# jorr3/Alphazero-4-player-chess

Measured on AMD Instinct MI355X. Metric: MCTS simulations/sec (whole node), 256 games×400 sims, 10-block ResNet, higher is better.
Workload: dtype fp16

## Files before the change

### alphazero-4-player-chess_amd/csrc/fpc_nn.h

```cpp
#pragma once
#include <hip/hip_runtime.h>

#include <algorithm>
#include <cstdlib>
#include <cstring>
#include <string>
#include <vector>

#include "fpc_tree_kernels.h"
#include "fpc_tower.h"
#include "fpc_towerw.h"

namespace fpc {

typedef __attribute__((ext_vector_type(8))) __bf16 bf16x8_t;
typedef __attribute__((ext_vector_type(8))) _Float16 f16x8_t;
typedef __attribute__((ext_vector_type(16))) float f32x16_t;
typedef __attribute__((ext_vector_type(4))) uint32_t u32x4_t;
typedef __attribute__((ext_vector_type(2))) uint32_t u32x2_t;
typedef __attribute__((ext_vector_type(4))) float f32x4_t;

template <int DT>
struct E16;
template <>
// ... 273 lines not shown
          if (q0 + 64 * u < chunks) {
            const u32x4_t x = xrow[q0 + 64 * u];
            a0 = Dot16<DT>::dot2(w[u][0], x[0], a0); a1 = Dot16<DT>::dot2(w[u][1], x[1], a1);
            a2 = Dot16<DT>::dot2(w[u][2], x[2], a2); a3 = Dot16<DT>::dot2(w[u][3], x[3], a3);
          }
        }
      }
      float a = (a0 + a1) + (a2 + a3);
      for (int off = 32; off >= 1; off >>= 1) a += __shfl_xor(a, off);
      if (lane == 0) ll[(size_t)g * FPC_MAX_MOVES + j] = bias[nsrc] + a;
    }
    p = pend;
  }
}

template <int DT>
__global__ void __launch_bounds__(64) k_value_tail(const uint16_t *Y, const float *w, float bias, int P, int R, int PP,
                                                   int n, float *out) {
  const int g = blockIdx.x;
  if (g >= n) return;
  const int lane = threadIdx.x & 63;
  float acc = 0.f;
  for (int idx = lane; idx < R * R * 32; idx += 64) {
    const int q = idx >> 5, ch = idx & 31;
    const long m = (long)g * PP + (q / R + 1) * P + (q % R + 1);
    acc += E16<DT>::to_f32(Y[m * 32 + ch]) * w[idx];
  }
  for (int off = 32; off >= 1; off >>= 1) acc += __shfl_xor(acc, off);
  if (lane == 0) out[g] = tanhf(acc + bias);
}

template <int DT>
__global__ void __launch_bounds__(64) k_nchw_to_grid(const float *x, int n, int R, int P, uint16_t *out) {
  const int g = blockIdx.x;
  if (g >= n) return;
  const int lane = threadIdx.x & 63, RR = R * R;
  for (int q = lane; q < RR; q += 64) {
    uint16_t *row = out + ((long)g * P * P + (q / R + 1) * P + (q % R + 1)) * 32;
    for (int c = 0; c < 32; ++c) row[c] = c < 24 ? E16<DT>::from_f32(x[((long)g * 24 + c) * RR + q]) : (uint16_t)0;
  }
}

struct BlobHeader {
  char magic[4];
  int32_t version, R, F, nblocks, dtype, A_ch, Np, Kp;
  int32_t fc_layout;
  int32_t pad[6];
};
static_assert(sizeof(BlobHeader) == 64, "header is 64 bytes");

struct ConvW {
  uint16_t *w = nullptr;
  float *b = nullptr;
  int cin = 0, cout_pad = 0;
};

struct NN {
  bool loaded = false;
  DevCfg dc{};
  int Gmax = 0, dtype = 0, F = 0, nblocks = 0, P = 0, PP = 0, Np = 0, Kp = 0, Mrows = 0, guard = 64, Gpad = 0;
  hipStream_t stream = nullptr;
  std::vector<void *> allocs;
  uint16_t *in16 = nullptr;
  uint16_t *act[3] = {nullptr, nullptr, nullptr};
  uint16_t *yv = nullptr;
  uint16_t *xfc = nullptr;
  float *d_logits = nullptr;
  float *d_stats = nullptr;
  float *d_value = nullptr;
  ConvW stem, pconv, vconv;
  std::vector<ConvW> c1, c2;
  uint16_t *fcw = nullptr;
  float *fcb = nullptr, *vw = nullptr;
  float *fc_part = nullptr;
  int fc_G1 = 0, fc_s1 = FC_SPLITK, fc_s2 = FC_SPLITK;
  int fc_layout = 1;
  int fc_gw = 256;
  unsigned char *towerW = nullptr;
  unsigned char *stemW = nullptr;
  float *towerB = nullptr;
  bool use_tower = false;
  int tower_waves = 8;
  bool tower_compact = true;
  int towerw_rows = 1;
  bool use_towerw = false;
  void (*mark_fn)(void *, int) = nullptr;
  void *mark_ctx = nullptr;
  float vb = 0.f;
  bool attr_conv[2][3] = {{false, false, false}, {false, false, false}}, attr_tower[2] = {false, false}, attr_towerw[2] = {false, false}, attr_fc[2] = {false, false}, attr_gemv = false;

  template <class T>
  int dmalloc(T **p, size_t count, std::string *err) {
    void *q = nullptr;
    if (hipMalloc(&q, count * sizeof(T)) != hipSuccess) { *err = "hipMalloc failed in NN (" + std::to_string(count * sizeof(T)) + " bytes)"; return FPC_ENOMEM; }
    (void)hipMemset(q, 0, count * sizeof(T));
    allocs.push_back(q);
    *p = (T *)q;
    return 0;
  }

  int init(const DevCfg &c, int max_games, int nn_dtype, hipStream_t s, std::string *) {
    dc = c; Gmax = max_games; dtype = nn_dtype ? 1 : 0; stream = s;
    P = c.R + 2; PP = P * P;
    Mrows = ((max_games * PP + CONV_BM - 1) / CONV_BM) * CONV_BM;
    Gpad = ((max_games + 255) / 256) * 256;
    return 0;
  }
  void destroy() {
    for (void *p : allocs) (void)hipFree(p);
    allocs.clear();
    loaded = false;
    fcw2 = nullptr; d_ll = nullptr;
  }
  uint16_t *input16() { return in16 + (size_t)guard * 32; }
  const fpc_board *in_boards = nullptr;
  const int *in_leaf_slot = nullptr, *in_leaf_turn = nullptr;
  int in_board_stride = 0;
  bool takes_boards() const { return use_tower || use_towerw; }
  void set_board_input(const fpc_board *b, int stride, const int *slot, const int *turn) { in_boards = b; in_board_stride = stride; in_leaf_slot = slot; in_leaf_turn = turn; }
  uint16_t one16() const { return dtype ? 0x3C00 : 0x3F80; }
  float *logits() { return d_logits; }
  float *stats() { return d_stats; }
  float *value() { return d_value; }
  uint16_t *fcw2 = nullptr;
  float *d_ll = nullptr;
  float *legal_logits() { return d_ll; }

  static int plan_fcw(int Np, int Kp, int cus) {
    const int groups = Np / FCW_COLS, stages = Kp / 64;
    int best = 0;
    for (int sk = 1; sk <= 2 * FC_SPLITK && groups * sk <= cus; ++sk)
      if (stages % sk == 0 && stages / sk >= 4) best = sk;
    return best;
  }
  void plan_fc() {
    if (fc_layout == 2) { fc_G1 = Np / FCW_COLS; fc_s2 = fc_s1; return; }
    fc_s1 = FC_SPLITK;
    const int groups = Np / 256, ks = Kp / 16, mt = (Gmax + 255) / 256;
    fc_s2 = (ks % (2 * FC_SPLITK * 8) == 0 && ks / (2 * FC_SPLITK) / 4 >= 4) ? 2 * FC_SPLITK : FC_SPLITK;
    fc_G1 = groups;
    if (fc_s2 == FC_SPLITK) return;
    int cus = 256;
    hipDeviceProp_t prop;
    int dev = 0;
    (void)hipGetDevice(&dev);
    if (hipGetDeviceProperties(&prop, dev) == hipSuccess && prop.multiProcessorCount > 0) cus = prop.multiProcessorCount;
    long best = -1;
    std::vector<long> fin(cus);
    for (int g1 = groups; g1 >= 0; --g1) {
      std::fill(fin.begin(), fin.end(), 0L);
      for (int y = 0; y < mt; ++y)
        for (int id = 0, nb = g1 * FC_SPLITK + (groups - g1) * fc_s2; id < nb; ++id) {
          auto it = std::min_element(fin.begin(), fin.end());
          *it += id < g1 * FC_SPLITK ? 2 : 1;
        }
      const long span = *std::max_element(fin.begin(), fin.end());
      if (best < 0 || span < best) { best = span; fc_G1 = g1; }
    }
  }

  int load(const void *blob, uint64_t nbytes, std::string *err) {
    if (nbytes < sizeof(BlobHeader)) { *err = "weight blob too small"; return FPC_EWEIGHTS; }
    BlobHeader h;
    memcpy(&h, blob, sizeof(h));
    if (memcmp(h.magic, "FPCW", 4) || h.version != 3) { *err = "bad weight blob magic/version (this engine reads version 3; version 2 carried the retired 32x32x16 policy-Linear order: export again)"; return FPC_EWEIGHTS; }
    if (h.R != dc.R || h.A_ch != dc.A_ch) { *err = "weight blob is for a different board size"; return FPC_EWEIGHTS; }
    if (h.dtype != dtype) { *err = "weight blob dtype differs from engine nn_dtype"; return FPC_EWEIGHTS; }
    if (h.fc_layout < 1 || h.fc_layout > 2) { *err = "unknown policy-Linear weight layout in weight blob (1 = k_fc16, 2 = k_fcw)"; return FPC_EWEIGHTS; }
    if (h.F % 64 || h.F < 64 || h.F > 512 || h.nblocks < 0 || h.Np % (h.fc_layout == 2 ? FCW_COLS : 256) || h.Kp % 512 || h.Kp < 1024 || h.Np < dc.A || h.Kp < dc.A) {
      *err = "unsupported network shape in weight blob (hidden must be a multiple of 64, Np of 256 -- 384 for fc_layout 2 --, Kp of 512)";
      return FPC_EWEIGHTS;
    }
    int fcw_split = 0;
    if (h.fc_layout == 2) {
      int cus = 256, dev = 0;
      hipDeviceProp_t prop;
      (void)hipGetDevice(&dev);
      if (hipGetDeviceProperties(&prop, dev) == hipSuccess && prop.multiProcessorCount > 0) cus = prop.multiProcessorCount;
      fcw_split = plan_fcw(h.Np, h.Kp, cus);
      if (!fcw_split) { *err = "weight blob fc_layout 2 (k_fcw): no one-round K-split for this shape on this device; export with fc_layout 1"; return FPC_EWEIGHTS; }
    }
    destroy();
    F = h.F; nblocks = h.nblocks; Np = h.Np; Kp = h.Kp;
    fc_layout = h.fc_layout;
    fc_gw = fc_layout == 2 ? FCW_COLS : 256;
    if (fc_layout == 2) fc_s1 = fcw_split;
    const unsigned char *base = (const unsigned char *)blob;
    uint64_t off = sizeof(BlobHeader);
    int rc = 0;
    auto take = [&](void **dev, uint64_t bytes) -> int {
      off = (off + 63) & ~63ull;
      if (off + bytes > nbytes) { *err = "weight blob truncated"; return FPC_EWEIGHTS; }
      unsigned char *d = nullptr;
      if ((rc = dmalloc(&d, bytes, err))) return rc;
      if (hipMemcpy(d, base + off, bytes, hipMemcpyHostToDevice) != hipSuccess) { *err = "weight upload failed"; return FPC_ENODEVICE; }
      off += bytes;
      *dev = d;
      return 0;
    };
    auto conv = [&](ConvW &cw, int cin, int cout_pad) -> int {
      cw.cin = cin; cw.cout_pad = cout_pad;
      if ((rc = take((void **)&cw.w, (uint64_t)9 * cout_pad * cin * 2))) return rc;
      return take((void **)&cw.b, (uint64_t)cout_pad * 4);
    };
    const int Fp = (F + GEMM_BN - 1) / GEMM_BN * GEMM_BN;
    if ((rc = conv(stem, 32, Fp))) return rc;
    c1.assign(nblocks, ConvW()); c2.assign(nblocks, ConvW());
    for (int i = 0; i < nblocks; ++i) { if ((rc = conv(c1[i], F, Fp)) || (rc = conv(c2[i], F, Fp))) return rc; }
    if ((rc = conv(pconv, F, 128))) return rc;
    if ((rc = conv(vconv, F, 128))) return rc;
    if ((rc = take((void **)&fcw, (uint64_t)Np * Kp * 2)) || (rc = take((void **)&fcb, (uint64_t)Np * 4))) return rc;
    if ((rc = take((void **)&vw, (uint64_t)dc.RR * 32 * 4))) return rc;
    off = (off + 63) & ~63ull;
    if (off + 4 > nbytes) { *err = "weight blob truncated"; return FPC_EWEIGHTS; }
    memcpy(&vb, base + off, 4);
    const size_t rows = (size_t)Mrows + 2 * guard;
    if ((rc = dmalloc(&in16, rows * 32, err))) return rc;
    for (auto &a : act) if ((rc = dmalloc(&a, rows * F, err))) return rc;
    if ((rc = dmalloc(&yv, rows * 32, err))) return rc;
    if ((rc = dmalloc(&xfc, (size_t)Gpad * Kp, err))) return rc;
    if ((rc = dmalloc(&fc_part, (size_t)2 * FC_SPLITK * Gpad * Np, err))) return rc;
    plan_fc();
    if ((rc = dmalloc(&d_logits, (size_t)Gmax * dc.A, err))) return rc;
    if ((rc = dmalloc(&d_stats, (size_t)Gmax * SM_MAXCH * SM_REC, err))) return rc;
    if ((rc = dmalloc(&d_value, (size_t)Gmax, err))) return rc;
    use_tower = use_towerw = false;
    const bool dev = getenv("FPC_DEV_KNOBS") && atoi(getenv("FPC_DEV_KNOBS")) != 0;
    auto knob = [dev](const char *name, int dflt) { const char *v = dev ? getenv(name) : nullptr; return v ? atoi(v) : dflt; };
    const bool no_tower = knob("FPC_NO_TOWER", 0) != 0;
    tower_waves = knob("FPC_TOWER_WAVES", 8);
    tower_compact = knob("FPC_TOWER_COMPACT", 1) != 0;
    if (F == 256 && !no_tower) {
      use_towerw = true;
      towerw_rows = knob("FPC_TOWERW_ROWS", 1);
    } else if (F == 128 && !no_tower) {
      const int kw = knob("FPC_TOWERW", -1);
      use_towerw = kw < 0 ? dc.R != 14 : kw != 0;
      use_tower = !use_towerw;
    }
    const int layers = 2 * nblocks + 2;
    if (use_towerw) {
      const int slab = tww_slab(F), ksn = F / 32, tiles = F / 16;
      if ((rc = dmalloc(&towerW, ((size_t)layers * 9 * ksn + TWW_PAD_SLABS) * slab, err)) || (rc = dmalloc(&stemW, (size_t)9 * slab, err)) ||
          (rc = dmalloc(&towerB, (size_t)layers * 256, err))) return rc;
      auto prep = [&](const ConvW &cw, int layer) {
        hipLaunchKernelGGL(k_towerw_prep, dim3((9 * ksn * tiles * 64 + 255) / 256), dim3(256), 0, stream, (const uint16_t *)cw.w,
                           towerW + (size_t)layer * 9 * ksn * slab, 9, cw.cout_pad, F, tiles);
        (void)hipMemcpyAsync(towerB + (size_t)layer * 256, cw.b, (size_t)std::min(cw.cout_pad, F) * 4, hipMemcpyDeviceToDevice, stream);
      };
      for (int i = 0; i < nblocks; ++i) { prep(c1[i], 2 * i); prep(c2[i], 2 * i + 1); }
      prep(vconv, 2 * nblocks);
      prep(pconv, 2 * nblocks + 1);
      hipLaunchKernelGGL(k_towerw_prep, dim3((9 * tiles * 64 + 255) / 256), dim3(256), 0, stream, (const uint16_t *)stem.w, stemW, 9, stem.cout_pad, 32, tiles);
      if (hipStreamSynchronize(stream) != hipSuccess || hipGetLastError() != hipSuccess) { *err = "k_towerw_prep failed"; return FPC_ENODEVICE; }
    } else if (use_tower) {
      if ((rc = dmalloc(&towerW, (size_t)(layers * 9 + 3) * TW_TAP, err)) || (rc = dmalloc(&stemW, (size_t)9 * TW_STEM_TAP, err)) ||
          (rc = dmalloc(&towerB, (size_t)layers * 256, err))) return rc;
      auto prep = [&](const ConvW &cw, int layer) {
        hipLaunchKernelGGL(k_tower_prep, dim3((9 * 128 * 16 + 255) / 256), dim3(256), 0, stream, (const uint16_t *)cw.w,
                           towerW + (size_t)layer * 9 * TW_TAP, 9, 128);
        (void)hipMemcpyAsync(towerB + (size_t)layer * 256, cw.b, 128 * 4, hipMemcpyDeviceToDevice, stream);
      };
      for (int i = 0; i < nblocks; ++i) { prep(c1[i], 2 * i); prep(c2[i], 2 * i + 1); }
      prep(vconv, 2 * nblocks);
      prep(pconv, 2 * nblocks + 1);
      hipLaunchKernelGGL(k_tower_prep, dim3((9 * 128 * 4 + 255) / 256), dim3(256), 0, stream, (const uint16_t *)stem.w, stemW, 9, 32);
      if (hipStreamSynchronize(stream) != hipSuccess) { *err = "k_tower_prep failed"; return FPC_ENODEVICE; }
    }
    loaded = true;
    return 0;
  }

  template <int DT, int CINC>
  int launch_conv_c(const ConvArgs &g, int M, std::string *err) {
    constexpr int BKS = CINC < 64 ? CINC : 64;
    constexpr int IMG = (CONV_BM + 2 * CONV_HMAX) * CINC * 2;
    constexpr int lds = (IMG > CONV_BM * 64 * 4 ? IMG : CONV_BM * 64 * 4) + 3 * CONV_BN * BKS * 2 + CONV_BM;
    bool &attr = attr_conv[DT][CINC == 32 ? 0 : CINC == 64 ? 1 : 2];
    if (!attr) {
      (void)hipFuncSetAttribute(reinterpret_cast<const void *>(&k_conv3x3<DT, CINC>), hipFuncAttributeMaxDynamicSharedMemorySize, lds);
      attr = true;
    }
    dim3 grid(M / CONV_BM, g.cout_pad / CONV_BN), block(CONV_THREADS);
    hipLaunchKernelGGL((k_conv3x3<DT, CINC>), grid, block, lds, stream, g);
    const hipError_t le = hipGetLastError();
    if (le != hipSuccess) { *err = std::string("k_conv3x3 launch failed: ") + hipGetErrorString(le); return FPC_ENODEVICE; }
    return 0;
  }
  template <int DT>
  int launch_conv(const ConvArgs &g, int M, std::string *err) {
    if (g.P + 1 > CONV_HMAX) { *err = "board too large for the conv halo"; return FPC_EINVAL; }
    if (g.cin == 32) return launch_conv_c<DT, 32>(g, M, err);
    if (g.cin == 64) return launch_conv_c<DT, 64>(g, M, err);
    if (g.cin % 128 == 0) return launch_conv_c<DT, 128>(g, M, err);
    *err = "unsupported conv input width";
    return FPC_EINVAL;
  }

  template <int DT>
  int forward_t(int n, float *logits_out, float *value_out, std::string *err) {
    int rc;
    const int M = ((n * PP + CONV_BM - 1) / CONV_BM) * CONV_BM;
    auto conv = [&](const ConvW &cw, const uint16_t *in, int in_ld, const uint16_t *res, uint16_t *out, int out_ld, int n_valid, int mode) -> int {
      ConvArgs g{};
      g.X = in + (size_t)guard * in_ld; g.W = cw.w; g.bias = cw.b;
      g.Res = res ? res + (size_t)guard * out_ld : nullptr;
      g.out = mode == 1 ? out : out + (size_t)guard * out_ld;
      g.ldx = in_ld; g.ldo = out_ld; g.cin = cw.cin; g.cout_pad = cw.cout_pad;
      g.P = P; g.R = dc.R; g.PP = PP; g.n_valid = n_valid; g.m_valid = n; g.mode = mode;
      return launch_conv<DT>(g, M, err);
    };
    int cur = 0;
    if (use_tower || use_towerw) {
      TowerArgs t{};
      t.boards = in_boards; t.leaf_slot = in_leaf_slot; t.leaf_turn = in_leaf_turn; t.board_stride = in_board_stride; t.one16 = one16();
      in_boards = nullptr;
      t.in16 = in16 + (size_t)guard * 32; t.Wstem = stemW; t.bstem = stem.b; t.Wt = towerW; t.bt = towerB;
      t.xfc = xfc; t.vw = vw; t.value = value_out; t.vb = vb;
      t.L = 2 * nblocks; t.P = P; t.R = dc.R; t.PP = PP; t.NR = PP - P; t.T0 = (P + 1) / 16; t.n_games = n; t.Kp = Kp; t.A_ch = dc.A_ch; t.rules = dc.rules;
#if defined(TW_STAMPS) || defined(TWW_STAMPS)
      static unsigned long long *d_stamps = nullptr;
      if (!d_stamps) { (void)hipMalloc(&d_stamps, 2 * 8 * 16 * 8); }
      (void)hipMemsetAsync(d_stamps, 0, 2 * 8 * 16 * 8, stream);
      t.stamps = d_stamps;
#endif
      const int mt = dc.R <= 8 ? 3 : dc.R <= 11 ? 5 : 7;
      bool &attr = attr_tower[DT];
      if (!attr) {
        (void)hipFuncSetAttribute(reinterpret_cast<const void *>(&k_tower<DT, 3, false, 4>), hipFuncAttributeMaxDynamicSharedMemorySize, TW_LDS);
        (void)hipFuncSetAttribute(reinterpret_cast<const void *>(&k_tower<DT, 5, false, 4>), hipFuncAttributeMaxDynamicSharedMemorySize, TW_LDS);
        (void)hipFuncSetAttribute(reinterpret_cast<const void *>(&k_tower<DT, 7, false, 4>), hipFuncAttributeMaxDynamicSharedMemorySize, TW_LDS);
        (void)hipFuncSetAttribute(reinterpret_cast<const void *>(&k_tower<DT, 7, true, 4>), hipFuncAttributeMaxDynamicSharedMemorySize, TW_LDS);
        (void)hipFuncSetAttribute(reinterpret_cast<const void *>(&k_tower<DT, 7, true, 8>), hipFuncAttributeMaxDynamicSharedMemorySize, TW_LDS);
        (void)hipFuncSetAttribute(reinterpret_cast<const void *>(&k_tower<DT, 3, false, 8>), hipFuncAttributeMaxDynamicSharedMemorySize, TW_LDS);
        (void)hipFuncSetAttribute(reinterpret_cast<const void *>(&k_tower<DT, 5, false, 8>), hipFuncAttributeMaxDynamicSharedMemorySize, TW_LDS);
        (void)hipFuncSetAttribute(reinterpret_cast<const void *>(&k_tower<DT, 7, false, 8>), hipFuncAttributeMaxDynamicSharedMemorySize, TW_LDS);
        (void)hipFuncSetAttribute(reinterpret_cast<const void *>(&k_towerc<DT>), hipFuncAttributeMaxDynamicSharedMemorySize, TW_LDS);
        attr = true;
      }
      if (use_towerw) {
        bool &aw = attr_towerw[DT];
        if (!aw) {
#define FPC_TWW_ATTR(F_, MT_) (void)hipFuncSetAttribute(reinterpret_cast<const void *>(&k_towerw<DT, F_, MT_>), hipFuncAttributeMaxDynamicSharedMemorySize, tww_lds(F_))
#define FPC_TWW_ATTRS(F_) FPC_TWW_ATTR(F_, 2); FPC_TWW_ATTR(F_, 3); FPC_TWW_ATTR(F_, 4); FPC_TWW_ATTR(F_, 5); FPC_TWW_ATTR(F_, 6); FPC_TWW_ATTR(F_, 7)
          FPC_TWW_ATTRS(256); FPC_TWW_ATTRS(128);
#define FPC_TWW_ATTR1(F_, MT_) (void)hipFuncSetAttribute(reinterpret_cast<const void *>(&k_towerw<DT, F_, MT_, true>), hipFuncAttributeMaxDynamicSharedMemorySize, tww_lds(F_))
          FPC_TWW_ATTR1(128, 4); FPC_TWW_ATTR1(256, 4); FPC_TWW_ATTR1(256, 6); FPC_TWW_ATTR1(256, 7); FPC_TWW_ATTR1(256, 8);
          FPC_TWW_ATTR1(256, 9); FPC_TWW_ATTR1(256, 11); FPC_TWW_ATTR1(256, 13);
#undef FPC_TWW_ATTR1
          aw = true;
        }
        const int mtw = tww_mt(dc.R);
        if (mtw < 2 || mtw > 7) { *err = "k_towerw: board size outside 8..14"; return FPC_EINVAL; }
#define FPC_TWW_GO(F_, MT_) hipLaunchKernelGGL((k_towerw<DT, F_, MT_>), dim3(n), dim3(TWW_THREADS), tww_lds(F_), stream, t)
#define FPC_TWW_GOS(F_) switch (mtw) { case 2: FPC_TWW_GO(F_, 2); break; case 3: FPC_TWW_GO(F_, 3); break; case 4: FPC_TWW_GO(F_, 4); break; \
                                       case 5: FPC_TWW_GO(F_, 5); break; case 6: FPC_TWW_GO(F_, 6); break; default: FPC_TWW_GO(F_, 7); break; }
        const int tiles = tww_tiles(dc.R);
        const bool onerow = tiles <= 4 || (F == 256 && towerw_rows != 2);
#define FPC_TWW_GO1(F_, MT_) hipLaunchKernelGGL((k_towerw<DT, F_, MT_, true>), dim3(n), dim3(TWW_THREADS), tww_lds(F_), stream, t)
        if (onerow && F == 128) FPC_TWW_GO1(128, 4);
        else if (onerow) {
          switch (tiles) {
            case 4: FPC_TWW_GO1(256, 4); break;   case 6: FPC_TWW_GO1(256, 6); break;   case 7: FPC_TWW_GO1(256, 7); break;
            case 8: FPC_TWW_GO1(256, 8); break;   case 9: FPC_TWW_GO1(256, 9); break;   case 11: FPC_TWW_GO1(256, 11); break;
            default: FPC_TWW_GO1(256, 13); break;
          }
        } else if (F == 256) { FPC_TWW_GOS(256) } else { FPC_TWW_GOS(128) }
#undef FPC_TWW_GO1
#undef FPC_TWW_GOS
#undef FPC_TWW_GO
      } else if (mt == 3 && tower_waves == 8) hipLaunchKernelGGL((k_tower<DT, 3, false, 8>), dim3(n), dim3(512), TW_LDS, stream, t);
      else if (mt == 3) hipLaunchKernelGGL((k_tower<DT, 3, false, 4>), dim3(n), dim3(256), TW_LDS, stream, t);
      else if (mt == 5 && tower_waves == 8) hipLaunchKernelGGL((k_tower<DT, 5, false, 8>), dim3(n), dim3(512), TW_LDS, stream, t);
      else if (mt == 5) hipLaunchKernelGGL((k_tower<DT, 5, false, 4>), dim3(n), dim3(256), TW_LDS, stream, t);
      else if (P != 16 && tower_waves == 8) hipLaunchKernelGGL((k_tower<DT, 7, false, 8>), dim3(n), dim3(512), TW_LDS, stream, t);
      else if (P != 16) hipLaunchKernelGGL((k_tower<DT, 7, false, 4>), dim3(n), dim3(256), TW_LDS, stream, t);
      else if (tower_waves == 8 && tower_compact && dc.R == 14) hipLaunchKernelGGL((k_towerc<DT>), dim3(n), dim3(512), TW_LDS, stream, t);
      else if (tower_waves == 8) hipLaunchKernelGGL((k_tower<DT, 7, true, 8>), dim3(n), dim3(512), TW_LDS, stream, t);
      else hipLaunchKernelGGL((k_tower<DT, 7, true, 4>), dim3(n), dim3(256), TW_LDS, stream, t);
      const hipError_t le = hipGetLastError();
      if (le != hipSuccess) { *err = std::string("k_tower launch failed: ") + hipGetErrorString(le); return FPC_ENODEVICE; }
#if defined(TW_STAMPS) || defined(TWW_STAMPS)
      if (getenv("FPC_TW_STAMPS_FILE")) {
        unsigned long long h[2 * 8 * 16];
        (void)hipStreamSynchronize(stream);
        (void)hipMemcpy(h, t.stamps, sizeof(h), hipMemcpyDeviceToHost);
        if (FILE *f = fopen(getenv("FPC_TW_STAMPS_FILE"), "w")) {
          for (int i = 0; i < 2 * 8 * 16; ++i) fprintf(f, "%llu%c", h[i], i % 16 == 15 ? '\n' : ' ');
          fclose(f);
        }
      }
#endif
    } else if ((rc = conv(stem, in16, 32, nullptr, act[0], F, F, 0))) return rc;
    const bool fused = use_tower || use_towerw;
    for (int i = 0; i < nblocks && !fused; ++i) {
      const int t1 = (cur + 1) % 3, t2 = (cur + 2) % 3;
      if ((rc = conv(c1[i], act[cur], F, nullptr, act[t1], F, F, 0))) return rc;
      if ((rc = conv(c2[i], act[t1], F, act[cur], act[t2], F, F, 0))) return rc;
      cur = t2;
    }
    if (!fused) {
      if ((rc = conv(pconv, act[cur], F, nullptr, xfc, Kp, dc.A_ch, 1))) return rc;
      if ((rc = conv(vconv, act[cur], F, nullptr, yv, 32, 24, 0))) return rc;
    }
    if (mark_fn) mark_fn(mark_ctx, 2);
#if defined(TW_STRIP) && (TW_STRIP & 128)
    if (false) {
#else
    if (logits_out) {
#endif
      FcArgs f{};
      f.X = xfc; f.Wf = fcw; f.part = fc_part; f.Kp = Kp; f.Np = Np; f.ksteps = Kp / 16; f.Mtot = Gpad;
      f.G1 = fc_G1; f.s1 = fc_s1; f.s2 = fc_s2;
      const int mtiles = (n + 255) / 256;
      const int blocks = fc_G1 * fc_s1 + (Np / fc_gw - fc_G1) * fc_s2;
      bool &fattr = attr_fc[DT];
      if (!fattr) {
        (void)hipFuncSetAttribute(reinterpret_cast<const void *>(&k_fc16<DT>), hipFuncAttributeMaxDynamicSharedMemorySize, FC_LDS);
        (void)hipFuncSetAttribute(reinterpret_cast<const void *>(&k_fcw<DT>), hipFuncAttributeMaxDynamicSharedMemorySize, FCW_LDS);
        fattr = true;
      }
      if (fc_layout == 2) hipLaunchKernelGGL((k_fcw<DT>), dim3(blocks, mtiles), dim3(FC_THREADS), FCW_LDS, stream, f);
      else hipLaunchKernelGGL((k_fc16<DT>), dim3(blocks, mtiles), dim3(FC_THREADS), FC_LDS, stream, f);
      hipLaunchKernelGGL(k_fc_reduce, dim3((dc.A / 4 + 255) / 256, n), dim3(256), 0, stream, (const float *)fc_part, (const float *)fcb,
                         fc_G1, fc_s1, fc_s2, fc_gw, Gpad, dc.A, n, skip_dense ? (float *)nullptr : logits_out, d_stats);
      const hipError_t le = hipGetLastError();
      if (le != hipSuccess) { *err = std::string("k_fc launch failed: ") + hipGetErrorString(le); return FPC_ENODEVICE; }
    }
    if (!fused) hipLaunchKernelGGL((k_value_tail<DT>), dim3(n), dim3(64), 0, stream, (const uint16_t *)(yv + (size_t)guard * 32),
                       (const float *)vw, vb, P, dc.R, PP, n, value_out);
    if (hipGetLastError() != hipSuccess) { *err = "k_value_tail launch failed"; return FPC_ENODEVICE; }
    return 0;
  }

  bool skip_dense = false;
  int forward(int n, bool dense_logits, std::string *err) {
    skip_dense = !dense_logits;
    const int rc = dtype ? forward_t<1>(n, d_logits, d_value, err) : forward_t<0>(n, d_logits, d_value, err);
    skip_dense = false;
    return rc;
  }
  static_assert(2 * FC_SPLITK <= LOGIT_MAX_SLABS, "logit_at() requests at most LOGIT_MAX_SLABS slabs per column");
  LogitSrc logit_src(bool dense) const {
    if (dense) return LogitSrc{d_logits, nullptr, nullptr, 0, 0, 0, 0, 256};
    return LogitSrc{nullptr, fc_part, fcb, fc_G1, fc_s1, fc_s2, Gpad, fc_gw};
  }
  int ensure_legal_head(std::string *err) {
    if (fcw2) return 0;
    if (Gmax > GEMV_MAXG) { *err = "legal-only policy head supports at most " + std::to_string(GEMV_MAXG) + " games per engine"; return FPC_EINVAL; }
    int rc;
    if ((rc = dmalloc(&fcw2, (size_t)Np * Kp, err)) || (rc = dmalloc(&d_ll, (size_t)Gmax * FPC_MAX_MOVES, err))) return rc;
    const long chunks = (long)Np * (Kp / 8);
    if (dtype) hipLaunchKernelGGL((k_fc_unfrag<1>), dim3((unsigned)((chunks + 255) / 256)), dim3(256), 0, stream, (const uint16_t *)fcw, fcw2, Np, Kp);
    else hipLaunchKernelGGL((k_fc_unfrag<0>), dim3((unsigned)((chunks + 255) / 256)), dim3(256), 0, stream, (const uint16_t *)fcw, fcw2, Np, Kp);
    if (hipGetLastError() != hipSuccess) { *err = "k_fc_unfrag launch failed"; return FPC_ENODEVICE; }
    return 0;
  }
  int forward_legal(int n, const Tree &t, std::string *err) {
    int rc = ensure_legal_head(err);
    if (rc) return rc;
// ... 27 lines not shown
```

### alphazero-4-player-chess_amd/csrc/fpc_tower.h

```cpp
#pragma once
#include <hip/hip_runtime.h>

#include <type_traits>

#include "fpc_tree_kernels.h"

namespace fpc {

typedef __attribute__((ext_vector_type(8))) __bf16 t_bf16x8;
typedef __attribute__((ext_vector_type(8))) _Float16 t_f16x8;
typedef __attribute__((ext_vector_type(4))) float t_f32x4;
typedef __attribute__((ext_vector_type(2))) float t_f32x2;
typedef __attribute__((ext_vector_type(4))) uint32_t t_u32x4;
typedef __attribute__((ext_vector_type(2))) uint32_t t_u32x2;
typedef __attribute__((ext_vector_type(2))) short t_i16x2;

template <int DT>
struct M16;
template <>
struct M16<0> {
  static __device__ __forceinline__ t_f32x4 mfma(t_u32x4 a, t_u32x4 b, t_f32x4 c) {
    return __builtin_amdgcn_mfma_f32_16x16x32_bf16(__builtin_bit_cast(t_bf16x8, a), __builtin_bit_cast(t_bf16x8, b), c, 0, 0, 0);
  }
  static __device__ __forceinline__ uint32_t pack2(float lo, float hi) {
// ... 43 lines not shown
  const int *leaf_slot, *leaf_turn;
  int board_stride;
  uint16_t one16;
  const uint16_t *in16;
  const unsigned char *Wstem;
  const float *bstem;
  const unsigned char *Wt;
  const float *bt;
  uint16_t *xfc;
  const float *vw;
  float *value;
  float vb;
  int L, P, R, PP, NR, T0, n_games, Kp, A_ch;
  int rules;
  unsigned long long *stamps;
};

__device__ __forceinline__ void tw_dma_8k(const unsigned char *gsrc_uniform, uint32_t lane_off, uint32_t lds_addr_uniform) {
  uint32_t keep;
  asm volatile(
      "s_mov_b32 %0, m0\n\ts_mov_b32 m0, %3\n\ts_nop 0\n\t"
      "global_load_lds_dwordx4 %1, %2\n\ts_add_u32 m0, m0, 0x400\n\tv_add_u32 %1, 0x400, %1\n\t"
      "global_load_lds_dwordx4 %1, %2\n\ts_add_u32 m0, m0, 0x400\n\tv_add_u32 %1, 0x400, %1\n\t"
      "global_load_lds_dwordx4 %1, %2\n\ts_add_u32 m0, m0, 0x400\n\tv_add_u32 %1, 0x400, %1\n\t"
      "global_load_lds_dwordx4 %1, %2\n\ts_add_u32 m0, m0, 0x400\n\tv_add_u32 %1, 0x400, %1\n\t"
      "global_load_lds_dwordx4 %1, %2\n\ts_add_u32 m0, m0, 0x400\n\tv_add_u32 %1, 0x400, %1\n\t"
      "global_load_lds_dwordx4 %1, %2\n\ts_add_u32 m0, m0, 0x400\n\tv_add_u32 %1, 0x400, %1\n\t"
      "global_load_lds_dwordx4 %1, %2\n\ts_add_u32 m0, m0, 0x400\n\tv_add_u32 %1, 0x400, %1\n\t"
      "global_load_lds_dwordx4 %1, %2\n\t"
      "s_mov_b32 m0, %0"
      : "=&s"(keep), "+v"(lane_off) : "s"(gsrc_uniform), "s"(lds_addr_uniform) : "memory", "scc");
}
__device__ __forceinline__ void tw_dma_4k(const unsigned char *gsrc_uniform, uint32_t lane_off, uint32_t lds_addr_uniform) {
  uint32_t keep;
  asm volatile(
      "s_mov_b32 %0, m0\n\ts_mov_b32 m0, %3\n\ts_nop 0\n\t"
      "global_load_lds_dwordx4 %1, %2\n\ts_add_u32 m0, m0, 0x400\n\tv_add_u32 %1, 0x400, %1\n\t"
      "global_load_lds_dwordx4 %1, %2\n\ts_add_u32 m0, m0, 0x400\n\tv_add_u32 %1, 0x400, %1\n\t"
      "global_load_lds_dwordx4 %1, %2\n\ts_add_u32 m0, m0, 0x400\n\tv_add_u32 %1, 0x400, %1\n\t"
      "global_load_lds_dwordx4 %1, %2\n\t"
      "s_mov_b32 m0, %0"
      : "=&s"(keep), "+v"(lane_off) : "s"(gsrc_uniform), "s"(lds_addr_uniform) : "memory", "scc");
}
template <int OFF>
__device__ __forceinline__ void tw_dma_piece(const unsigned char *gsrc_uniform, uint32_t lane_off) {
  asm volatile("global_load_lds_dwordx4 %0, %1 offset:%2" : : "v"(lane_off), "s"(gsrc_uniform), "i"(OFF) : "memory");
}
__device__ __forceinline__ void tw_set_m0(uint32_t lds_addr_uniform) {
  asm volatile("s_mov_b32 m0, %0\n\ts_nop 0" : : "s"(lds_addr_uniform) : "memory");
}
__device__ __forceinline__ void tw_dma_256(const unsigned char *gsrc_uniform, uint32_t lane_off, uint32_t lds_addr_uniform) {
  uint32_t keep;
  asm volatile("s_mov_b32 %0, m0\n\ts_mov_b32 m0, %3\n\ts_nop 0\n\tglobal_load_lds_dword %1, %2\n\ts_mov_b32 m0, %0"
               : "=&s"(keep) : "v"(lane_off), "s"(gsrc_uniform), "s"(lds_addr_uniform) : "memory");
}

#ifdef TW_STAMPS
#define TW_STAMP(GT, I)                                                                                       \
  do {                                                                                                        \
    if (g.stamps && blockIdx.x == 0 && ((GT) == TW_STAMPS || (GT) == TW_STAMPS + 1)) {                        \
      const unsigned long long t_ = __builtin_amdgcn_s_memtime();                                             \
      if (lane == 0) g.stamps[(((GT) - TW_STAMPS) * 8 + wave) * 16 + (I)] = t_;                               \
    }                                                                                                         \
  } while (0)
#else
#define TW_STAMP(GT, I) do {} while (0)
#endif
#ifndef TW_AHEAD
#define TW_AHEAD 2
#endif
#ifndef TW_LOADERS
#define TW_LOADERS 1
#endif
#ifndef TW_STAGGER
#define TW_STAGGER 3
#endif
#ifndef TW_STRIP
#define TW_STRIP 0
#endif
#ifndef TWC_LOADER_TILES
#define TWC_LOADER_TILES 6
#endif

template <int DT, int MT, bool FAST, int NW, int LOAD, bool CMP = false>
__device__ __forceinline__ void tw_body(const TowerArgs &g) {
  static_assert(!CMP || (!FAST && NW == 8 && TW_LOADERS == 1 && MT == (LOAD == 2 ? TWC_LOADER_TILES : 13 - TWC_LOADER_TILES)), "compact form: 8 waves, 13 row tiles");
  constexpr int CR = 14, CZ = 16;
  constexpr int TB0 = LOAD == 2 ? 0 : TWC_LOADER_TILES;
  constexpr int NT = NW * 64;
  constexpr int WN = NW / 2;
  constexpr int CT = 8 / WN;
  constexpr int PIECES = 4 * LOAD;
  constexpr int DMA_PER_WAVE = PIECES * 1024;
  constexpr int MID = PIECES == 8 ? 4096 : 0;
  constexpr bool STREAM = TW_AHEAD == 2 && !(TW_STAGGER != 0 && NW == 8 && TW_LOADERS == 1);
  constexpr int STAG = (NW == 8 && TW_LOADERS == 1 && LOAD == 0) ? TW_STAGGER : 0;
  extern __shared__ __attribute__((aligned(16))) unsigned char smem[];
  unsigned char *const img = smem + TW_IMG0;
  unsigned char *const ring = smem + TW_RING;
  const float *const biasbuf = reinterpret_cast<const float *>(smem + TW_BIAS);
  float *const vred = reinterpret_cast<float *>(smem + TW_VRED);
  fpc_board *const lboard = reinterpret_cast<fpc_board *>(smem + TW_BOARD);
  const int tid = threadIdx.x, lane = tid & 63;
  const int wave = __builtin_amdgcn_readfirstlane(tid >> 6);
  const int wm = wave / WN, wn = wave % WN;
  const int li = lane & 15, lq = lane >> 4;
  const int game = blockIdx.x;
  const int P = g.P, NR = g.NR;

  int slot = 0, rot_k = 0;
  if (g.boards) {
    slot = g.leaf_slot[game];
    if (slot < 0) return;
    rot_k = first_leaf_turn(g.leaf_slot, g.leaf_turn, g.n_games);
  }

  const int rbase = CMP ? CZ + TB0 * 16 + li : (g.T0 + wm * MT) * 16 + li;
  uint32_t inmask = 0;
#pragma unroll
  for (int mt = 0; mt < MT; ++mt) {
    const int r = rbase + 16 * mt;
    if (CMP) {
      if (r - CZ < CR * CR) inmask |= 1u << mt;
    } else {
      const int pi = r / P, pj = r - pi * P;
      if (r < g.PP && pi >= 1 && pi <= g.R && pj >= 1 && pj <= g.R) inmask |= 1u << mt;
    }
  }
  auto colmask = [](int mt, int dx) -> uint64_t {
    uint32_t m16 = 0;
    for (int i = 0; i < 16; ++i)
      if (dx != 0 && ((TB0 + mt) * 16 + i) % CR == (dx < 0 ? 0 : CR - 1)) m16 |= 1u << i;
    const uint32_t m32 = m16 * 0x10001u;
    return ((uint64_t)m32 << 32) | m32;
  };
  auto lane_select = [](uint32_t a, uint32_t b, uint64_t m) -> uint32_t {
    uint32_t r;
    asm("v_cndmask_b32_e64 %0, %1, %2, %3" : "=v"(r) : "v"(a), "v"(b), "s"(m));
    return r;
  };
  const int bq = (lq >> 1) * 256 + (lq & 1) * 128;
  const int apart = (li >> 3) * 2048 + (li & 7) * 16 + bq;
  const int apart_s = (li >> 3) * 512 + (li & 7) * 16 + bq;
  const int cb64 = wn * (CT * 16);
  const int cb16 = (wn & 1) * 16;
  const bool vactive = wn < 2;

  for (int c = tid; c < (TW_IMG0 + TW_IMG) / 16; c += NT) reinterpret_cast<t_u32x4 *>(smem)[c] = t_u32x4{0u, 0u, 0u, 0u};
  unsigned char *const enc = smem + TW_ENC;
  const int enc_bytes = CMP ? 240 * 64 : ((NR + 7) >> 3) * 512;
  for (int c = tid; c < enc_bytes / 16; c += NT) reinterpret_cast<t_u32x4 *>(enc)[c] = t_u32x4{0u, 0u, 0u, 0u};
  {
    const t_u32x4 *src = reinterpret_cast<const t_u32x4 *>(g.Wstem);
    t_u32x4 *dst = reinterpret_cast<t_u32x4 *>(ring);
    for (int c = tid; c < 9 * TW_STEM_TAP / 16; c += NT) dst[c] = src[c];
  }
  t_f32x4 bst[CT];
#pragma unroll
  for (int ct = 0; ct < CT; ++ct) bst[ct] = *reinterpret_cast<const t_f32x4 *>(g.bstem + cb64 + ct * 16 + 4 * lq);
  __syncthreads();
  if (g.boards) {
    constexpr int WPB = (int)(sizeof(fpc_board) / 4);
    if (tid < WPB) reinterpret_cast<uint32_t *>(lboard)[tid] =
        reinterpret_cast<const uint32_t *>(g.boards + (size_t)game * g.board_stride + slot)[tid];
    __syncthreads();
    if (g.rules & FPC_RULES_ROTATION) rot_k = lboard->turn;
    for (int r = tid; r < (CMP ? CR * CR : g.PP); r += NT) {
      const int pi = CMP ? r / CR + 1 : r / P, pj = CMP ? r % CR + 1 : r - pi * P;
      if (pi < 1 || pi > g.R || pj < 1 || pj > g.R) continue;
      const uint8_t p = lboard->sq[rot90_src(g.R, rot_k, pi - 1, pj - 1)];
      if (!present(p)) continue;
      const int plane = piece_plane(p, lboard->turn, g.rules);
      *reinterpret_cast<uint16_t *>(enc + tw_lay(4, CMP ? CZ + r : r, plane >> 3) + (plane & 7) * 2) = g.one16;
    }
  } else if (CMP) {
    const uint16_t *src = g.in16 + (size_t)game * g.PP * 32;
    for (int c = tid; c < CR * CR * 4; c += NT) {
      const int q = c >> 2, j = c & 3;
      *reinterpret_cast<t_u32x4 *>(enc + tw_lay(4, CZ + q, j)) =
// ... 59 lines not shown
  auto open_tap = [&](int T) {
    issue_bias(T);
    if (LOAD == 0) return;
    dsrc = g.Wt + (size_t)T * TW_TAP + lw * DMA_PER_WAVE + MID;
    tw_set_m0((uint32_t)__builtin_amdgcn_readfirstlane(TW_RING + (T % 3) * TW_TAP + lw * DMA_PER_WAVE + MID));
  };
  auto piece = [&](auto i_c) {
    constexpr int I = decltype(i_c)::value;
    if (LOAD != 0) tw_dma_piece<I * 1024 - MID>(dsrc, dma_lane);
  };
  issue_tap(0);
  issue_tap(1);
  if (STREAM) {
    open_tap(2);
    piece(std::integral_constant<int, 0>{});
    if (LOAD == 2) piece(std::integral_constant<int, 1>{});
  }

  unsigned char *const dummy = smem + TW_DUMMY + lane * 8;
  unsigned char *const wbase = img + (rbase >> 3) * 2048 + (rbase & 7) * 16 + wn * (CT * 256) + (lane >> 5) * 128 + ((lane >> 4) & 1) * 8;
  auto epilogue = [&](auto res_c) {
    constexpr int RES = decltype(res_c)::value;
    if (TW_STRIP & 16) return;
#pragma unroll
    for (int mt = 0; mt < MT; ++mt) {
      unsigned char *dst = ((inmask >> mt) & 1u) ? wbase + mt * 4096 : dummy;
#pragma unroll
      for (int ct = 0; ct < CT; ++ct) {
        t_f32x4 v = acc[mt][ct];
        if (RES == 2) {
          v[0] += M16<DT>::lo(res[mt][ct][0]); v[1] += M16<DT>::hi(res[mt][ct][0]);
          v[2] += M16<DT>::lo(res[mt][ct][1]); v[3] += M16<DT>::hi(res[mt][ct][1]);
        }
        const t_u32x2 pk = t_u32x2{tw_relu2(M16<DT>::pack2(v[0], v[1])), tw_relu2(M16<DT>::pack2(v[2], v[3]))};
        if (RES != 0) res[mt][ct] = pk;
        *reinterpret_cast<t_u32x2 *>(((inmask >> mt) & 1u) ? dst + ct * 256 : dst) = pk;
      }
      __builtin_amdgcn_sched_barrier(0);
    }
  };
  const std::integral_constant<int, 0> c0{};
  const std::integral_constant<int, 1> c1{};
  const std::integral_constant<int, 2> c2{};
  const std::integral_constant<int, 3> c3{};
  epilogue(c1);
  if (TW_STRIP & 32) { asm volatile("s_waitcnt vmcnt(0)" ::: "memory"); return; }
  if (STREAM) asm volatile("s_waitcnt vmcnt(%0)" ::"n"(PIECES + LOAD) : "memory");
  else asm volatile("s_waitcnt vmcnt(0)" ::: "memory");
  __syncthreads();

  t_u32x4 fa[2][CT], fb[2][MT];
  int gt = 0;
  const unsigned char *wslot;
  const unsigned char *bbase;
  const unsigned char *blast;
  int boff[FAST ? 1 : MT];
  auto set_tap = [&](int tap, int cb) {
    wslot = ring + (gt % 3) * TW_TAP + cb * 256 + apart;
    const int shift = (tap / 3 - 1) * P + (tap % 3 - 1);
    if (FAST) {
      const int r = rbase + shift;
      bbase = img + (r >> 3) * 2048 + (r & 7) * 16 + bq;
      int rl = r + 16 * (MT - 1);
      rl = rl >= NR ? rl - NR : rl;
      blast = img + (rl >> 3) * 2048 + (rl & 7) * 16 + bq;
    } else if (CMP) {
      const int dx = tap % 3 - 1;
      const int r = rbase + (tap / 3 - 1) * CR + dx;
      const uint32_t zoff = (r & 7) * 16 + bq;
      const uint32_t b0 = (r >> 3) * 2048 + zoff;
#pragma unroll
      for (int mt = 0; mt < MT; ++mt) {
        const uint64_t m = dx < 0 ? colmask(mt, -1) : dx > 0 ? colmask(mt, 1) : 0ull;
        boff[mt] = (int)lane_select(b0 + mt * 4096, zoff, m);
      }
    } else {
#pragma unroll
      for (int mt = 0; mt < MT; ++mt) {
        const int r = brow(mt, shift);
        boff[mt] = (r >> 3) * 2048 + (r & 7) * 16 + bq;
      }
    }
  };
  auto bptr = [&](int mt) -> const unsigned char * {
    if (FAST) return mt == MT - 1 ? blast : bbase + mt * 4096;
    return img + boff[mt];
  };
  auto kstep = [&](auto mode_c, auto buf_c, auto ksn_c, auto bias_c, const t_f32x4 *b4, auto q_c) {
    constexpr int MODE = decltype(mode_c)::value, B = decltype(buf_c)::value, KSN = decltype(ksn_c)::value;
    constexpr bool BIAS = decltype(bias_c)::value != 0;
    constexpr int N = B ^ 1, Q = decltype(q_c)::value;
    if (!(TW_STRIP & 2)) {
#pragma unroll
      for (int ct = 0; ct < CT; ++ct) fa[N][ct] = *reinterpret_cast<const t_u32x4 *>(wslot + ct * 4096 + KSN * 512);
      fb[N][0] = *reinterpret_cast<const t_u32x4 *>(bptr(0) + KSN * 512);
    }
    __builtin_amdgcn_sched_barrier(0);
#pragma unroll
    for (int mt = 0; mt < MT; ++mt) {
      if (TW_STRIP & 1) {
        if (BIAS) {
#pragma unroll
          for (int ct = 0; ct < (MODE == 0 ? CT : 1); ++ct) acc[mt][ct] = b4[ct];
        }
        asm volatile("" : "+v"(fa[B][0]), "+v"(fb[B][mt]));
      } else if (MODE == 0) {
#pragma unroll
        for (int ct = 0; ct < CT; ++ct) acc[mt][ct] = M16<DT>::mfma(fa[B][ct], fb[B][mt], BIAS ? b4[ct] : acc[mt][ct]);
      } else if (NW == 4 || vactive) {
        acc[mt][0] = M16<DT>::mfma(fa[B][0], fb[B][mt], BIAS ? b4[0] : acc[mt][0]);
      }
      __builtin_amdgcn_sched_barrier(0);
      if (mt + 1 < MT && !(TW_STRIP & 2)) {
        fb[N][mt + 1] = *reinterpret_cast<const t_u32x4 *>(bptr(mt + 1) + KSN * 512);
        __builtin_amdgcn_sched_barrier(0);
      }
      if (STREAM && LOAD != 0) {
        if (mt == (LOAD == 2 ? MT / 3 : MT / 2)) piece(std::integral_constant<int, LOAD * Q>{});
        if (LOAD == 2 && mt == (2 * MT) / 3) piece(std::integral_constant<int, LOAD * Q + 1>{});
        __builtin_amdgcn_sched_barrier(0);
      }
    }
  };
  auto load_b0 = [&]() {
#pragma unroll
    for (int mt = 0; mt < MT; ++mt) fb[0][mt] = *reinterpret_cast<const t_u32x4 *>(bptr(mt));
  };
  auto run_layer = [&](auto mode_c, const int layer, const int cb, const int cb_next) {
    constexpr int MODE = decltype(mode_c)::value;
    t_f32x4 b4[CT];
    {
      const float *bl = biasbuf + (layer & 1) * 256 + cb + 4 * lq;
#pragma unroll
      for (int ct = 0; ct < (MODE == 0 ? CT : 1); ++ct) b4[ct] = *reinterpret_cast<const t_f32x4 *>(bl + ct * 16);
    }
    if (STAG == 3 && !(TW_STRIP & 8)) __syncthreads();
    kstep(mode_c, c0, c1, c1, b4, c1);
#pragma unroll 1
    for (int tap = 0; tap < 9; ++tap) {
      if (STAG == 2) {
        TW_STAMP(gt, 3);
        __syncthreads();
        TW_STAMP(gt, 4);
      }
      TW_STAMP(gt, 0);
      kstep(mode_c, c1, c2, c0, b4, c2);
      TW_STAMP(gt, 1);
      if (STAG == 1) __syncthreads();
      kstep(mode_c, c0, c3, c0, b4, c3);
      TW_STAMP(gt, 2);
      if (!STAG) {
        if (STREAM) asm volatile("s_waitcnt vmcnt(%0)" ::"n"(PIECES) : "memory");
        else asm volatile("s_waitcnt vmcnt(0)" ::: "memory");
        TW_STAMP(gt, 3);
        if (!(TW_STRIP & 8)) __syncthreads();
        TW_STAMP(gt, 4);
        if (STREAM) open_tap(gt + 3);
        else if (gt + 2 < total) issue_tap(gt + 2);
        TW_STAMP(gt, 5);
      }
      ++gt;
      set_tap(tap == 8 ? 0 : tap + 1, tap == 8 ? cb_next : cb);
      TW_STAMP(gt - 1, 6);
      kstep(mode_c, c1, c0, c0, b4, c0);
      TW_STAMP(gt - 1, 7);
      if (STAG == 3 && tap < 8 && !(TW_STRIP & 8)) __syncthreads();
      if (tap < 8) kstep(mode_c, c0, c1, c0, b4, c1);
      TW_STAMP(gt - 1, 8);
    }
  };

  set_tap(0, cb64);
#pragma unroll
  for (int ct = 0; ct < CT; ++ct) fa[0][ct] = *reinterpret_cast<const t_u32x4 *>(wslot + ct * 4096);
  load_b0();
  const int nblocks = g.L / 2;
#pragma unroll 1
  for (int blk = 0; blk < nblocks; ++blk) {
    run_layer(c0, 2 * blk, cb64, cb64);
    epilogue(c0);
    __syncthreads();
    load_b0();
    run_layer(c0, 2 * blk + 1, cb64, blk + 1 == nblocks ? cb16 : cb64);
    epilogue(c2);
    __syncthreads();
    load_b0();
  }
  float vpart = 0.f;
  {
    run_layer(c1, g.L, cb16, cb64);
#pragma unroll
    for (int mt = 0; mt < MT; ++mt) {
      const int r = rbase + 16 * mt;
      const int pi = r / P, pj = r - pi * P;
      const bool in = ((inmask >> mt) & 1u) && (NW == 4 || vactive);
      const int qp = !in ? 0 : CMP ? r - CZ : (pi - 1) * g.R + (pj - 1);
      const t_f32x4 w4 = *reinterpret_cast<const t_f32x4 *>(g.vw + qp * 32 + cb16 + 4 * lq);
#pragma unroll
      for (int j = 0; j < 4; ++j) {
        float v = acc[mt][0][j];
        v = v > 0.f ? v : 0.f;
        vpart += in ? v * w4[j] : 0.f;
      }
    }
  }
  run_layer(c0, g.L + 1, cb64, cb64);
  epilogue(c0);
  __syncthreads();

  if (!(TW_STRIP & 64)) {
    const int cpr = g.A_ch / 8;
    for (int c = tid; c < (CMP ? CR * CR : g.PP) * 16; c += NT) {
      const int j = c & 15;
      if (j >= cpr) continue;
      int r = c >> 4, q = r;
      if (CMP) r += CZ;
      else {
        const int pi = r / P, pj = r - pi * P;
        if (pi < 1 || pi > g.R || pj < 1 || pj > g.R) continue;
        q = (pi - 1) * g.R + (pj - 1);
      }
      *reinterpret_cast<t_u32x4 *>(g.xfc + (size_t)game * g.Kp + (size_t)q * g.A_ch + j * 8) =
          *reinterpret_cast<const t_u32x4 *>(img + tw_lay(16, r, j));
    }
  }
  for (int off = 32; off >= 1; off >>= 1) vpart += __shfl_xor(vpart, off);
  if (lane == 0) vred[wave] = vpart;
  __syncthreads();
  if (tid == 0) g.value[game] = tanhf(g.vb + ((vred[0] + vred[1]) + (vred[WN] + vred[WN + 1])));
  asm volatile("s_waitcnt vmcnt(0)" ::: "memory");
}

template <int DT, int MT, bool FAST, int NW>
__global__ void __launch_bounds__(NW * 64, NW / 4) k_tower(TowerArgs g) {
  if (NW == 8 && TW_LOADERS == 1) {
    if (__builtin_amdgcn_readfirstlane(threadIdx.x >> 6) < 4) tw_body<DT, MT, FAST, NW, 2>(g);
    else tw_body<DT, MT, FAST, NW, 0>(g);
  } else {
    tw_body<DT, MT, FAST, NW, NW == 4 ? 2 : 1>(g);
  }
}

template <int DT>
__global__ void __launch_bounds__(512, 2) k_towerc(TowerArgs g) {
  if (__builtin_amdgcn_readfirstlane(threadIdx.x >> 6) < 4) tw_body<DT, TWC_LOADER_TILES, false, 8, 2, true>(g);
  else tw_body<DT, 13 - TWC_LOADER_TILES, false, 8, 0, true>(g);
}

__global__ void __launch_bounds__(256) k_tower_prep(const uint16_t *W, unsigned char *out, int taps, int cin) {
  const int CH = cin / 8;
  const long c = (long)blockIdx.x * 256 + threadIdx.x;
  if (c >= (long)taps * 128 * CH) return;
  const int tap = (int)(c / (128 * CH)), rem = (int)(c % (128 * CH)), row = rem / CH, j = rem % CH;
  *reinterpret_cast<t_u32x4 *>(out + (size_t)tap * 128 * cin * 2 + tw_lay(CH, row, j)) =
      *reinterpret_cast<const t_u32x4 *>(W + ((size_t)tap * 128 + row) * cin + j * 8);
}

}
```

Before: 486,000.

## Add tap-specialised unrolled inner loop to compact tower kernel

Adds a templated variant of the compact residual-tower kernel in which the 9-tap conv loop is restructured into a 3x3 loop with compile-time tap position. Weight-slot and B-offset selection become constant per tap, weight DMA uses precomputed source/destination pointers, and next-layer bias is prefetched by DMA. A separate stagger setting is also introduced for this path. The aim is to cut per-tap address arithmetic and scalar overhead in the hot loop. The cost is more code size and register pressure, plus a new code path that could diverge from the original.

```diff
diff --git a/alphazero-4-player-chess_amd/csrc/fpc_nn.h b/alphazero-4-player-chess_amd/csrc/fpc_nn.h
--- a/alphazero-4-player-chess_amd/csrc/fpc_nn.h
+++ b/alphazero-4-player-chess_amd/csrc/fpc_nn.h
@@ -379,6 +379,7 @@
   bool use_tower = false;
   int tower_waves = 8;
   bool tower_compact = true;
+  bool tower_taploop = true;
   int towerw_rows = 1;
   bool use_towerw = false;
   void (*mark_fn)(void *, int) = nullptr;
@@ -527,6 +528,7 @@
     const bool no_tower = knob("FPC_NO_TOWER", 0) != 0;
     tower_waves = knob("FPC_TOWER_WAVES", 8);
     tower_compact = knob("FPC_TOWER_COMPACT", 1) != 0;
+    tower_taploop = knob("FPC_TOWER_TAPLOOP", 1) != 0;
     if (F == 256 && !no_tower) {
       use_towerw = true;
       towerw_rows = knob("FPC_TOWERW_ROWS", 1);
@@ -632,7 +634,8 @@
         (void)hipFuncSetAttribute(reinterpret_cast<const void *>(&k_tower<DT, 3, false, 8>), hipFuncAttributeMaxDynamicSharedMemorySize, TW_LDS);
         (void)hipFuncSetAttribute(reinterpret_cast<const void *>(&k_tower<DT, 5, false, 8>), hipFuncAttributeMaxDynamicSharedMemorySize, TW_LDS);
         (void)hipFuncSetAttribute(reinterpret_cast<const void *>(&k_tower<DT, 7, false, 8>), hipFuncAttributeMaxDynamicSharedMemorySize, TW_LDS);
-        (void)hipFuncSetAttribute(reinterpret_cast<const void *>(&k_towerc<DT>), hipFuncAttributeMaxDynamicSharedMemorySize, TW_LDS);
+        (void)hipFuncSetAttribute(reinterpret_cast<const void *>(&k_towerc<DT, false>), hipFuncAttributeMaxDynamicSharedMemorySize, TW_LDS);
+        (void)hipFuncSetAttribute(reinterpret_cast<const void *>(&k_towerc<DT, true>), hipFuncAttributeMaxDynamicSharedMemorySize, TW_LDS);
         attr = true;
       }
       if (use_towerw) {
@@ -672,7 +675,8 @@
       else if (mt == 5) hipLaunchKernelGGL((k_tower<DT, 5, false, 4>), dim3(n), dim3(256), TW_LDS, stream, t);
       else if (P != 16 && tower_waves == 8) hipLaunchKernelGGL((k_tower<DT, 7, false, 8>), dim3(n), dim3(512), TW_LDS, stream, t);
       else if (P != 16) hipLaunchKernelGGL((k_tower<DT, 7, false, 4>), dim3(n), dim3(256), TW_LDS, stream, t);
-      else if (tower_waves == 8 && tower_compact && dc.R == 14) hipLaunchKernelGGL((k_towerc<DT>), dim3(n), dim3(512), TW_LDS, stream, t);
+      else if (tower_waves == 8 && tower_compact && dc.R == 14 && tower_taploop) hipLaunchKernelGGL((k_towerc<DT, true>), dim3(n), dim3(512), TW_LDS, stream, t);
+      else if (tower_waves == 8 && tower_compact && dc.R == 14) hipLaunchKernelGGL((k_towerc<DT, false>), dim3(n), dim3(512), TW_LDS, stream, t);
       else if (tower_waves == 8) hipLaunchKernelGGL((k_tower<DT, 7, true, 8>), dim3(n), dim3(512), TW_LDS, stream, t);
       else hipLaunchKernelGGL((k_tower<DT, 7, true, 4>), dim3(n), dim3(256), TW_LDS, stream, t);
       const hipError_t le = hipGetLastError();
diff --git a/alphazero-4-player-chess_amd/csrc/fpc_tower.h b/alphazero-4-player-chess_amd/csrc/fpc_tower.h
--- a/alphazero-4-player-chess_amd/csrc/fpc_tower.h
+++ b/alphazero-4-player-chess_amd/csrc/fpc_tower.h
@@ -149,9 +149,14 @@
 #define TWC_LOADER_TILES 6
 #endif
 
-template <int DT, int MT, bool FAST, int NW, int LOAD, bool CMP = false>
+#ifndef TWC_STAGGER
+#define TWC_STAGGER 2
+#endif
+
+template <int DT, int MT, bool FAST, int NW, int LOAD, bool CMP = false, bool TU = false>
 __device__ __forceinline__ void tw_body(const TowerArgs &g) {
   static_assert(!CMP || (!FAST && NW == 8 && TW_LOADERS == 1 && MT == (LOAD == 2 ? TWC_LOADER_TILES : 13 - TWC_LOADER_TILES)), "compact form: 8 waves, 13 row tiles");
+  static_assert(!TU || (CMP && TW_STAGGER != 0 && TWC_STAGGER >= 1 && TWC_STAGGER <= 3), "tap-specialised loop: compact form with the burst stream");
   constexpr int CR = 14, CZ = 16;
   constexpr int TB0 = LOAD == 2 ? 0 : TWC_LOADER_TILES;
   constexpr int NT = NW * 64;
@@ -161,7 +166,7 @@
   constexpr int DMA_PER_WAVE = PIECES * 1024;
   constexpr int MID = PIECES == 8 ? 4096 : 0;
   constexpr bool STREAM = TW_AHEAD == 2 && !(TW_STAGGER != 0 && NW == 8 && TW_LOADERS == 1);
-  constexpr int STAG = (NW == 8 && TW_LOADERS == 1 && LOAD == 0) ? TW_STAGGER : 0;
+  constexpr int STAG = (NW == 8 && TW_LOADERS == 1 && LOAD == 0) ? (TU ? TWC_STAGGER : TW_STAGGER) : 0;
   extern __shared__ __attribute__((aligned(16))) unsigned char smem[];
   unsigned char *const img = smem + TW_IMG0;
   unsigned char *const ring = smem + TW_RING;
@@ -387,6 +392,24 @@
       }
     }
   };
+  const unsigned char *wrow = nullptr, *wrow2 = nullptr;
+  auto set_wrow = [&](int cb) {
+    int o = cb * 256 + apart, o2 = o + 2 * TW_TAP;
+    asm volatile("" : "+v"(o2));
+    wrow = ring + o;
+    wrow2 = ring + o2;
+  };
+  int rrow = rbase - CR;
+  auto set_tap_u = [&](auto xn_c) {
+    constexpr int XN = decltype(xn_c)::value;
+    wslot = XN == 2 ? wrow2 : wrow + XN * TW_TAP;
+    const int r = rrow + (XN - 1);
+    const uint32_t zoff = (r & 7) * 16 + bq;
+    const uint32_t b0 = (r >> 3) * 2048 + zoff;
+#pragma unroll
+    for (int mt = 0; mt < MT; ++mt)
+      boff[mt] = XN == 1 ? (int)(b0 + mt * 4096) : (int)lane_select(b0 + mt * 4096, zoff, colmask(mt, XN - 1));
+  };
   auto bptr = [&](int mt) -> const unsigned char * {
     if (FAST) return mt == MT - 1 ? blast : bbase + mt * 4096;
     return img + boff[mt];
@@ -431,8 +454,47 @@
 #pragma unroll
     for (int mt = 0; mt < MT; ++mt) fb[0][mt] = *reinterpret_cast<const t_u32x4 *>(bptr(mt));
   };
+  const unsigned char *usrc = g.Wt + (size_t)TW_TAP + lw * DMA_PER_WAVE;
+  const uint32_t udst = (uint32_t)__builtin_amdgcn_readfirstlane(TW_RING + lw * DMA_PER_WAVE);
+  auto tap_u = [&](auto mode_c, auto x_c, const t_f32x4 *b4, const int dy, const int cb_next) {
+    constexpr int X = decltype(x_c)::value;
+    if (STAG == 2) {
+      TW_STAMP(gt, 3);
+      __syncthreads();
+      TW_STAMP(gt, 4);
+    }
+    TW_STAMP(gt, 0);
+    kstep(mode_c, c1, c2, c0, b4, c2);
+    TW_STAMP(gt, 1);
+    if (STAG == 1) __syncthreads();
+    kstep(mode_c, c0, c3, c0, b4, c3);
+    TW_STAMP(gt, 2);
+    if (!STAG) {
+      asm volatile("s_waitcnt vmcnt(0)" ::: "memory");
+      TW_STAMP(gt, 3);
+      if (!(TW_STRIP & 8)) __syncthreads();
+      TW_STAMP(gt, 4);
+      if (LOAD != 0 && !(TW_STRIP & 4)) {
+        usrc += TW_TAP;
+        tw_dma_8k(usrc, dma_lane, udst + ((X + 2) % 3) * TW_TAP);
+      }
+      TW_STAMP(gt, 5);
+    }
+    ++gt;
+    if (X == 2) {
+      rrow = dy == 1 ? rbase - CR : rrow + CR;
+      if (dy == 1) set_wrow(cb_next);
+    }
+    set_tap_u(std::integral_constant<int, (X + 1) % 3>{});
+    TW_STAMP(gt - 1, 6);
+    kstep(mode_c, c1, c0, c0, b4, c0);
+    TW_STAMP(gt - 1, 7);
+  };
   auto run_layer = [&](auto mode_c, const int layer, const int cb, const int cb_next) {
     constexpr int MODE = decltype(mode_c)::value;
+    if (TU && wave < 4 && layer + 1 < g.L + 2)
+      tw_dma_256(reinterpret_cast<const unsigned char *>(g.bt + (size_t)(layer + 1) * 256 + wave * 64), (uint32_t)lane * 4u,
+                 (uint32_t)__builtin_amdgcn_readfirstlane(TW_BIAS + (((layer + 1) & 1) * 256 + wave * 64) * 4));
     t_f32x4 b4[CT];
     {
       const float *bl = biasbuf + (layer & 1) * 256 + cb + 4 * lq;
@@ -441,6 +503,26 @@
     }
     if (STAG == 3 && !(TW_STRIP & 8)) __syncthreads();
     kstep(mode_c, c0, c1, c1, b4, c1);
+    if (TU) {
+#pragma unroll 1
+      for (int dy = -1;; ++dy) {
+        tap_u(mode_c, c0, b4, dy, cb_next);
+        if (STAG == 3 && !(TW_STRIP & 8)) __syncthreads();
+        kstep(mode_c, c0, c1, c0, b4, c1);
+        TW_STAMP(gt - 1, 8);
+        tap_u(mode_c, c1, b4, dy, cb_next);
+        if (STAG == 3 && !(TW_STRIP & 8)) __syncthreads();
+        kstep(mode_c, c0, c1, c0, b4, c1);
+        TW_STAMP(gt - 1, 8);
+        tap_u(mode_c, c2, b4, dy, cb_next);
+        if (dy == 1) break;
+        if (STAG == 3 && !(TW_STRIP & 8)) __syncthreads();
+        kstep(mode_c, c0, c1, c0, b4, c1);
+        TW_STAMP(gt - 1, 8);
+      }
+      TW_STAMP(gt - 1, 8);
+      return;
+    }
 #pragma unroll 1
     for (int tap = 0; tap < 9; ++tap) {
       if (STAG == 2) {
@@ -475,7 +557,12 @@
     }
   };
 
-  set_tap(0, cb64);
+  if (TU) {
+    set_wrow(cb64);
+    set_tap_u(c0);
+  } else {
+    set_tap(0, cb64);
+  }
 #pragma unroll
   for (int ct = 0; ct < CT; ++ct) fa[0][ct] = *reinterpret_cast<const t_u32x4 *>(wslot + ct * 4096);
   load_b0();
@@ -546,10 +633,10 @@
   }
 }
 
-template <int DT>
+template <int DT, bool TU>
 __global__ void __launch_bounds__(512, 2) k_towerc(TowerArgs g) {
-  if (__builtin_amdgcn_readfirstlane(threadIdx.x >> 6) < 4) tw_body<DT, TWC_LOADER_TILES, false, 8, 2, true>(g);
-  else tw_body<DT, 13 - TWC_LOADER_TILES, false, 8, 0, true>(g);
+  if (__builtin_amdgcn_readfirstlane(threadIdx.x >> 6) < 4) tw_body<DT, TWC_LOADER_TILES, false, 8, 2, true, TU>(g);
+  else tw_body<DT, 13 - TWC_LOADER_TILES, false, 8, 0, true, TU>(g);
 }
 
 __global__ void __launch_bounds__(256) k_tower_prep(const uint16_t *W, unsigned char *out, int taps, int cin) {
```

Result: faster. 495,200 (median of 6 runs) (+1.9%).
